# FreditorK/Tensor-Train-Interior-Point-Method

Measured on AMD Instinct MI355X. Metric: sec/IPM-iter (AMEn KKT solve), maxcut dim=10 r=1; MFMA util% on core-contract, lower is better.
Workload: dtype f64

## Files before the change

### tensor-train-interior-point-method_amd/csrc/ttk_dense.hip

```cpp
#include <hip/hip_runtime.h>

#include "ttk_common.h"
#include "ttk_internal.h"

namespace {

constexpr int NB = 32;
constexpr int GT = 32, GK = 16;

typedef double double4_t __attribute__((ext_vector_type(4)));

template <bool TA, bool TB>
__global__ __launch_bounds__(256) void gemm_strided_kernel(const double *__restrict__ A, int lda,
                                                           const double *__restrict__ B, int ldb,
                                                           double *__restrict__ C, int ldc, int M, int N, int K,
                                                           double alpha, double beta, int lower_only) {
  const int n0 = blockIdx.x * GT, m0 = blockIdx.y * GT;
  if (lower_only && n0 > m0 + GT - 1) return;
  __shared__ double As[GK][GT + 1];
  __shared__ double Bs[GK][GT + 1];
  const int tid = threadIdx.x, lane = tid & 63, wid = tid >> 6;
  const int wr = wid >> 1, wc = wid & 1;
  const int l_mn = tid & 31, l_k = tid >> 5;
  const bool am = m0 + l_mn < M, bn = n0 + l_mn < N;
// ... 82 lines not shown
}

__global__ __launch_bounds__(256) void panel_trsm_kernel(double *A, int n, int k0, int kb, const int *status) {
  __shared__ double Ls[NB][NB + 1];
  if (*status) return;
  const int tid = threadIdx.x;
  ttk::staged_copy<4>(kb * kb, tid, 256, [&](int e) { return A[(int64_t)(k0 + e / kb) * n + k0 + e % kb]; },
                      [&](int e, double v) { Ls[e / kb][e % kb] = v; });
  __syncthreads();
  const int r = k0 + kb + blockIdx.x * 256 + tid;
  if (r >= n) return;
  double *a = A + (int64_t)r * n + k0;
  double x[NB];
#pragma unroll
  for (int j = 0; j < NB; ++j) x[j] = j < kb ? a[j] : 0.0;
#pragma unroll
  for (int j = 0; j < NB; ++j) {
    if (j < kb) {
      double s = x[j];
#pragma unroll
      for (int c = 0; c < NB; ++c)
        if (c < j) s -= x[c] * Ls[j][c];
      x[j] = s / Ls[j][j];
    }
  }
#pragma unroll
  for (int j = 0; j < NB; ++j)
    if (j < kb) a[j] = x[j];
}

__global__ __launch_bounds__(256) void zero_upper_kernel(double *A, int n, const int *status) {
  if (*status) return;
  const int64_t e = blockIdx.x * (int64_t)256 + threadIdx.x;
  if (e >= (int64_t)n * n) return;
  const int i = (int)(e / n), c = (int)(e % n);
  if (c > i) A[e] = 0.0;
}

__global__ __launch_bounds__(256) void trsm_diag_kernel(const double *__restrict__ L, int n, double *B, int nrhs,
                                                        int ldb, int r0, int kb, int trans) {
  __shared__ double Ls[NB][NB + 1];
  const int tid = threadIdx.x;
  ttk::staged_copy<4>(
      kb * kb, tid, 256,
      [&](int e) {
        const int i = e / kb, j = e - i * kb;
        return trans ? L[(int64_t)(r0 + j) * n + r0 + i] : L[(int64_t)(r0 + i) * n + r0 + j];
      },
      [&](int e, double v) { Ls[e / kb][e % kb] = v; });
  __syncthreads();
  const int c = blockIdx.x * 256 + tid;
  if (c >= nrhs) return;
  double x[NB];
#pragma unroll
  for (int j = 0; j < NB; ++j) x[j] = j < kb ? B[(int64_t)(r0 + j) * ldb + c] : 0.0;
  if (!trans) {
#pragma unroll
    for (int j = 0; j < NB; ++j) {
      if (j < kb) {
        double s = x[j];
#pragma unroll
        for (int q = 0; q < NB; ++q)
          if (q < j) s -= Ls[j][q] * x[q];
        x[j] = s / Ls[j][j];
      }
    }
  } else {
#pragma unroll
    for (int jj = NB - 1; jj >= 0; --jj) {
      if (jj < kb) {
        double s = x[jj];
#pragma unroll
        for (int q = 0; q < NB; ++q)
          if (q > jj && q < kb) s -= Ls[jj][q] * x[q];
        x[jj] = s / Ls[jj][jj];
      }
    }
  }
#pragma unroll
  for (int j = 0; j < NB; ++j)
    if (j < kb) B[(int64_t)(r0 + j) * ldb + c] = x[j];
}



__global__ __launch_bounds__(256) void colsum_kernel(const double *__restrict__ A, int n, double *__restrict__ out) {
  const int c = blockIdx.x * 256 + threadIdx.x;
  if (c >= n) return;
  out[c] = ttk::sum_ahead<8>(n, [&](int r) { return fabs(A[(int64_t)r * n + c]); }, 0.0);
}

__device__ __forceinline__ void panel_row_update(double *__restrict__ pi, const double *__restrict__ prow, int c,
                                                 int kb, double inv) {
  const double l = pi[c] * inv;
  pi[c] = l;
#pragma unroll 8
  for (int cc = c + 1; cc < kb; ++cc) pi[cc] -= l * prow[cc];
}

__global__ __launch_bounds__(1024) void getf2_panel_kernel(double *A, int n, int k0, int kb, int *piv, int *status) {
  __shared__ double wv[16];
  __shared__ int wi[16];
  __shared__ int s_p;
  const int tid = threadIdx.x, lane = tid & 63, wid = tid >> 6;
  for (int c = 0; c < kb; ++c) {
    const int j = k0 + c;
    double best = -1.0;
    int bi = j;
    for (int i = j + tid; i < n; i += 1024) {
      const double v = fabs(A[(int64_t)i * n + j]);
      if (v > best) {
        best = v;
        bi = i;
      }
    }
    ttk::wave_argmax(best, bi);
    if (lane == 0) {
      wv[wid] = best;
      wi[wid] = bi;
    }
    __syncthreads();
    if (tid == 0) {
      double b = wv[0];
      int p = wi[0];
      for (int w = 1; w < 16; ++w)
        if (wv[w] > b || (wv[w] == b && wi[w] < p)) {
          b = wv[w];
          p = wi[w];
        }
      s_p = p;
      piv[j] = p;
    }
    __syncthreads();
    const int p = s_p;
    if (p != j && tid < kb) {
      double *a = A + (int64_t)j * n + k0 + tid, *b = A + (int64_t)p * n + k0 + tid;
      const double t = *a;
      *a = *b;
      *b = t;
    }
    __syncthreads();
    const double d = A[(int64_t)j * n + j];
    if (d == 0.0) {
      if (tid == 0 && *status == 0) *status = j + 1;
      continue;
    }
    const double inv = 1.0 / d;
    const double *prow = A + (int64_t)j * n + k0;
    for (int i = j + 1 + tid; i < n; i += 1024) panel_row_update(A + (int64_t)i * n + k0, prow, c, kb, inv);
    __syncthreads();
  }
}

__global__ __launch_bounds__(1024) void getf2_panel_lds_kernel(double *A, int n, int k0, int kb, int *piv,
                                                               int *status) {
  extern __shared__ double P[];
  __shared__ double wv[16];
  __shared__ int wi[16];
  __shared__ int s_p;
  const int tid = threadIdx.x, lane = tid & 63, wid = tid >> 6, nt = blockDim.x, nw = nt >> 6;
  const int rows = n - k0, ld = kb + 1;
  ttk::staged_copy<8>(rows * kb, tid, nt, [&](int e) { return A[(int64_t)(k0 + e / kb) * n + k0 + e % kb]; },
                      [&](int e, double v) { P[(e / kb) * ld + e % kb] = v; });
  __syncthreads();
  for (int c = 0; c < kb; ++c) {
    double best = -1.0;
// ... 592 lines not shown
        hipLaunchKernelGGL((getf2_panel_reg_kernel<8, 3>), dim3(1), dim3(1024), 0, st, A, n, k0, kb, piv, status);
      else
        hipLaunchKernelGGL((getf2_panel_reg_kernel<8, 4>), dim3(1), dim3(1024), 0, st, A, n, k0, kb, piv, status);
    } else if (pshm <= 150000) {
      if (pshm > 65536)
        (void)hipFuncSetAttribute(reinterpret_cast<const void *>(getf2_panel_lds_kernel),
                                  hipFuncAttributeMaxDynamicSharedMemorySize, (int)pshm);
      const int ntp = g_lu_panel_narrow ? ((n - k0 + 63) / 64 * 64 < 1024 ? (n - k0 + 63) / 64 * 64 : 1024) : 1024;
      hipLaunchKernelGGL(getf2_panel_lds_kernel, dim3(1), dim3(ntp), pshm, st, A, n, k0, kb, piv, status);
    } else {
      hipLaunchKernelGGL(getf2_panel_kernel, dim3(1), dim3(1024), 0, st, A, n, k0, kb, piv, status);
    }
    const int rest = n - k0 - kb;
    if (g_lu_swap_u12) {
      if (n - kb > 0)
        hipLaunchKernelGGL(lu_swap_u12_kernel, dim3((n - kb + 255) / 256), dim3(256), 0, st, A, n, k0, kb, piv);
    } else {
      hipLaunchKernelGGL(laswp_kernel, dim3((n + 255) / 256), dim3(256), 0, st, A, n, k0, kb, piv);
      if (rest > 0)
        hipLaunchKernelGGL(lu_u12_kernel, dim3((rest + 255) / 256), dim3(256), 0, st, A, n, k0, kb);
    }
    if (rest > 0) {
      dim3 grid((rest + GT - 1) / GT, (rest + GT - 1) / GT);
      hipLaunchKernelGGL((gemm_strided_kernel<false, false>), grid, dim3(256), 0, st,
                         A + (int64_t)(k0 + kb) * n + k0, n, A + (int64_t)k0 * n + k0 + kb, n,
                         A + (int64_t)(k0 + kb) * n + k0 + kb, n, rest, rest, kb, -1.0, 1.0, 0);
    }
    TTK_LAUNCH_CHECK();
    k0 += kb;
  }
  if (want_rcond == 1) return lu_rcond_launch(st, A, n, piv, colsum, status, rcond);
  return TTK_OK;
}

int lu_rcond_launch(hipStream_t st, const double *LU, int n, const int *piv, const double *colsum, const int *status,
                    double *rcond) {
  const size_t shm_perm = 3 * (size_t)n * sizeof(double) + 2 * (size_t)n * sizeof(int);
  const int use_perm = shm_perm <= 140000;
  const size_t shm = use_perm ? shm_perm : 2 * (size_t)n * sizeof(double) + (size_t)n * sizeof(int);
  if (shm > 65536)
    (void)hipFuncSetAttribute(reinterpret_cast<const void *>(lu_rcond_kernel),
                              hipFuncAttributeMaxDynamicSharedMemorySize, (int)shm);
  const int exact = ttk::ctx().knob[TTK_KNOB_RCOND_EXACT] != 0;
  hipLaunchKernelGGL(lu_rcond_kernel, dim3(1), dim3(1024), shm, st, LU, n, piv, colsum, status, rcond, use_perm,
                     exact);
  TTK_LAUNCH_CHECK();
  return TTK_OK;
}

int lu_solve_cols(hipStream_t st, const double *LU, int n, const int *piv, double *B, int nrhs, int ldb) {
  const size_t shm = (size_t)n * (sizeof(double) + sizeof(int));
  if (shm > 65536)
    (void)hipFuncSetAttribute(reinterpret_cast<const void *>(lu_solve_cols_kernel),
                              hipFuncAttributeMaxDynamicSharedMemorySize, (int)shm);
  hipLaunchKernelGGL(lu_solve_cols_kernel, dim3(nrhs), dim3(1024), shm, st, LU, n, piv, B, ldb);
  TTK_LAUNCH_CHECK();
  return TTK_OK;
}


int cholesky_blocked(hipStream_t st, double *A, int n, int *status) {
  TTK_HIP(hipMemsetAsync(status, 0, sizeof(int), st));
  for (int k0 = 0; k0 < n; k0 += NB) {
    const int kb = n - k0 < NB ? n - k0 : NB;
    hipLaunchKernelGGL(potf2_block_kernel, dim3(1), dim3(256), 0, st, A, n, k0, kb, status);
    const int rest = n - k0 - kb;
    if (rest > 0) {
      hipLaunchKernelGGL(panel_trsm_kernel, dim3((rest + 255) / 256), dim3(256), 0, st, A, n, k0, kb, status);
      double *L21 = A + (int64_t)(k0 + kb) * n + k0;
      double *A22 = A + (int64_t)(k0 + kb) * n + k0 + kb;
      dim3 grid((rest + GT - 1) / GT, (rest + GT - 1) / GT);
      hipLaunchKernelGGL((gemm_strided_kernel<false, true>), grid, dim3(256), 0, st, L21, n, L21, n, A22, n, rest,
                         rest, kb, -1.0, 1.0, 1);
    }
    TTK_LAUNCH_CHECK();
  }
  hipLaunchKernelGGL(zero_upper_kernel, dim3((unsigned)(((int64_t)n * n + 255) / 256)), dim3(256), 0, st, A, n,
                     status);
  TTK_LAUNCH_CHECK();
  return TTK_OK;
}

int trsm_blocked(hipStream_t st, const double *L, int n, double *B, int nrhs, int ldb, int trans) {
  for (int s = 0; s < n; s += NB) {
    const int kb = n - s < NB ? n - s : NB;
    const int r0 = trans ? n - s - kb : s;
    hipLaunchKernelGGL(trsm_diag_kernel, dim3((nrhs + 255) / 256), dim3(256), 0, st, L, n, B, nrhs, ldb, r0, kb,
                       trans);
    const int rest = n - s - kb;
    if (rest > 0) {
      dim3 grid((nrhs + GT - 1) / GT, (rest + GT - 1) / GT);
      if (!trans) {
        hipLaunchKernelGGL((gemm_strided_kernel<false, false>), grid, dim3(256), 0, st,
                           L + (int64_t)(r0 + kb) * n + r0, n, B + (int64_t)r0 * ldb, ldb,
                           B + (int64_t)(r0 + kb) * ldb, ldb, rest, nrhs, kb, -1.0, 1.0, 0);
      } else {
        hipLaunchKernelGGL((gemm_strided_kernel<true, false>), grid, dim3(256), 0, st, L + (int64_t)r0 * n, n,
                           B + (int64_t)r0 * ldb, ldb, B, ldb, rest, nrhs, kb, -1.0, 1.0, 0);
      }
    }
    TTK_LAUNCH_CHECK();
  }
  return TTK_OK;
}

}
```

### tensor-train-interior-point-method_amd/csrc/ttk_host.hip

```cpp
#include <cmath>
#include <tuple>
#include <cstring>
#include <vector>

#include "ttk_common.h"
#include "ttk_internal.h"

namespace {

struct Scratch {
  hipStream_t st;
  std::vector<void *> ptrs;
  double *base = nullptr;
  int64_t cap = 0, used = 0;
  static int64_t slot(int64_t n) { return ((n > 0 ? n : 1) + 31) & ~(int64_t)31; }
  explicit Scratch(hipStream_t s, int64_t capacity = 0) : st(s) {
    void *p = nullptr;
    if (capacity > 0 && hipMallocAsync(&p, (size_t)capacity * sizeof(double), st) == hipSuccess) {
      ptrs.push_back(p);
      base = static_cast<double *>(p);
      cap = capacity;
    }
  }
  double *get(int64_t n) {
// ... 67 lines not shown
}

View v3(const double *p, int64_t a, int64_t b, int64_t c) { return View{p, 3, {a, b, c}, {b * c, c, 1}}; }

int einsum_out(hipStream_t st, const char *eq, std::initializer_list<View> ops, double *out, int ond,
               const int64_t *ost, double alpha, double beta) {
  int64_t d[1 + 8 * 10 + 2 + 8];
  int k = 0;
  d[k++] = (int64_t)ops.size();
  for (const View &o : ops) {
    d[k++] = reinterpret_cast<int64_t>(o.p);
    d[k++] = o.nd;
    for (int i = 0; i < o.nd; ++i) d[k++] = o.sh[i];
    for (int i = 0; i < o.nd; ++i) d[k++] = o.st[i];
  }
  d[k++] = 1;
  d[k++] = ond;
  for (int i = 0; i < ond; ++i) d[k++] = ost[i];
  return ttk_einsum(st, eq, d, out, alpha, beta);
}

}

extern "C" {

int ttk_dense_schur_solve(ttk_ctx ctx, int64_t r, int64_t n, int64_t R, const ttk_local_block *blk,
                          const double *rhs, const double *inv_I, double *sol, double *rcond_out) {
  ttk::CtxScope scope(ctx);
  hipStream_t st = ttk::ctx().stream;
  if (rcond_out) *rcond_out = NAN;
  const int64_t m = r * n * R;
  if (r < 1 || n < 1 || R < 1 || !blk || !rhs || !inv_I || !sol || m > (1 << 20)) {
    ttk::set_error("ttk_dense_schur_solve: bad arguments");
    return TTK_ERR_ARG;
  }
  static const char *ASSEMBLE = "lsr,smnS,LSR->lmLrnR", *APPLY = "lsr,smnS,LSR,rnR->lmL",
                    *APPLY_T = "lsr,smnS,LSR,lmL->rnR", *MATMUL = "ik,kj->ij";
  enum { B00, B01, B21, B22 };
  auto ops3 = [&](int b) {
    const ttk_local_block &q = blk[b];
    return std::make_tuple(v3(q.L, r, q.s, r),
                           View{q.A, 4, {q.s, n, n, q.S}, {q.a_strides[0], q.a_strides[1], q.a_strides[2], q.a_strides[3]}},
                           v3(q.R, R, q.S, R));
  };
  Scratch sc(st, 7 * Scratch::slot(m) + 5 * Scratch::slot(m * m) + Scratch::slot(2 * m + 16) + Scratch::slot(m / 2 + 1));
  double *rd = sc.get(m), *rc = sc.get(m), *rp = sc.get(m), *LXI = sc.get(m * m), *Leq = sc.get(m * m),
         *LZ = sc.get(m * m), *t = sc.get(m), *bvec = sc.get(m), *T1 = sc.get(m * m), *Am = sc.get(m * m),
         *t2 = sc.get(m), *t3 = sc.get(m), *work = sc.get(2 * m + 16);
  int *piv = reinterpret_cast<int *>(sc.get(m / 2 + 1));
  if (!rd || !rc || !rp || !LXI || !Leq || !LZ || !t || !bvec || !T1 || !Am || !t2 || !t3 || !work || !piv) {
    ttk::set_error("ttk_dense_schur_solve: scratch allocation failed");
    return TTK_ERR_HIP;
  }
  const int64_t sh3[3] = {r, n, R}, st_blk[3] = {3 * n * R, R, 1}, st_c[3] = {n * R, R, 1};
  const int64_t out6[6] = {n * R * m, R * m, m, n * R, R, 1};
  const int64_t mm[2] = {m, m}, s_mat[2] = {m, 1}, s_row[2] = {0, 1}, out2[2] = {1, 1};
  auto col = [&](int j) { return rhs + j * n * R; };
  int rc_ = TTK_OK;
#define STEP(x)              \
  do {                       \
    if (rc_ == TTK_OK) rc_ = (x); \
  } while (0)
  STEP(ttk_copy_nd(st, col(1), rd, 3, sh3, st_blk, st_c, 1.0, 0.0));
  STEP(ttk_copy_nd(st, col(2), rc, 3, sh3, st_blk, st_c, 1.0, 0.0));
  STEP(ttk_copy_nd(st, col(0), rp, 3, sh3, st_blk, st_c, 1.0, 0.0));
  {
    auto [a, b, c] = ops3(B22);
    STEP(einsum(st, ASSEMBLE, {a, b, c}, LXI));
  }
  STEP(ttk_mul_nd(st, LXI, inv_I, LXI, 2, mm, s_mat, s_row, s_mat, 1.0, 0.0));
  {
    auto [a, b, c] = ops3(B01);
    STEP(einsum(st, ASSEMBLE, {a, b, c}, Leq));
  }
  {
    auto [a, b, c] = ops3(B21);
    STEP(einsum(st, ASSEMBLE, {a, b, c}, LZ));
  }
  if (rc_) return rc_;
  rc_ = ttk_cholesky_sync(st, LZ, (int)m);
  if (rc_) return rc_;
  STEP(hipMemcpyAsync(t, rc, m * sizeof(double), hipMemcpyDeviceToDevice, st) ? TTK_ERR_HIP : 0);
  STEP(einsum_out(st, MATMUL, {mat(LXI, m, m), mat(rd, m, 1)}, t, 2, out2, -1.0, 1.0));
  STEP(ttk_trsm_lower(st, LZ, (int)m, t, 1, 1, 0));
  STEP(ttk_trsm_lower(st, LZ, (int)m, t, 1, 1, 1));
  STEP(hipMemcpyAsync(bvec, rp, m * sizeof(double), hipMemcpyDeviceToDevice, st) ? TTK_ERR_HIP : 0);
  STEP(einsum_out(st, MATMUL, {mat(Leq, m, m), mat(t, m, 1)}, bvec, 2, out2, -1.0, 1.0));
  STEP(ttk_trsm_lower(st, LZ, (int)m, LXI, (int)m, (int)m, 0));
  STEP(ttk_trsm_lower(st, LZ, (int)m, LXI, (int)m, (int)m, 1));
  STEP(einsum(st, MATMUL, {mat(LXI, m, m), View{Leq, 2, {m, m}, {1, m}}}, T1));
  STEP(einsum(st, MATMUL, {mat(Leq, m, m), mat(T1, m, m)}, Am));
  {
    auto [a, b, c] = ops3(B00);
    STEP(einsum_out(st, ASSEMBLE, {a, b, c}, Am, 6, out6, 1.0, 1.0));
  }
  STEP(ttk_add_diag(st, Am, (int)m, (int)m, 1e-11));
  if (rc_) return rc_;
  int forked = 0;
  rc_ = ttk::lu_factor_fork_rcond(st, Am, (int)m, piv, work, &forked);
  if (rc_) return rc_;
  STEP(ttk_lu_solve(st, Am, (int)m, piv, bvec, 1, 1));
  double *s0 = sol, *s1 = sol + n * R, *s2 = sol + 2 * n * R;
  STEP(ttk_copy_nd(st, bvec, s0, 3, sh3, st_c, st_blk, 1.0, 0.0));
  STEP(hipMemcpyAsync(t2, rd, m * sizeof(double), hipMemcpyDeviceToDevice, st) ? TTK_ERR_HIP : 0);
  {
    auto [a, b, c] = ops3(B01);
    const View x{s0, 3, {r, n, R}, {st_blk[0], st_blk[1], st_blk[2]}};
    STEP(einsum_out(st, APPLY_T, {a, b, c, x}, t2, 3, st_c, -1.0, 1.0));
  }
  STEP(ttk_mul_nd(st, t2, inv_I, s2, 3, sh3, st_c, st_c, st_blk, 1.0, 0.0));
  STEP(hipMemcpyAsync(t3, rc, m * sizeof(double), hipMemcpyDeviceToDevice, st) ? TTK_ERR_HIP : 0);
  {
    auto [a, b, c] = ops3(B22);
    const View x{s2, 3, {r, n, R}, {st_blk[0], st_blk[1], st_blk[2]}};
    STEP(einsum_out(st, APPLY, {a, b, c, x}, t3, 3, st_c, -1.0, 1.0));
  }
  STEP(ttk_trsm_lower(st, LZ, (int)m, t3, 1, 1, 0));
  STEP(ttk_trsm_lower(st, LZ, (int)m, t3, 1, 1, 1));
  STEP(ttk_copy_nd(st, t3, s1, 3, sh3, st_c, st_blk, 1.0, 0.0));
#undef STEP
  if (forked && ttk::lu_rcond_join(st)) return TTK_ERR_HIP;
  int lu_info = 0;
  double rcond = 0.0;
  if (hipMemcpyAsync(&lu_info, ttk::ctx().status, sizeof(int), hipMemcpyDeviceToHost, st) ||
      hipMemcpyAsync(&rcond, ttk::ctx().rcond, sizeof(double), hipMemcpyDeviceToHost, st))
    return TTK_ERR_HIP;
  ttk::note_sync();
  if (hipStreamSynchronize(st)) return TTK_ERR_HIP;
  if (rcond_out) *rcond_out = rcond;
  if (lu_info) {
    ttk::set_error("Matrix is singular (zero pivot at %d).", lu_info);
    return TTK_ERR_SINGULAR;
  }
  if (rcond < 0.5 * 2.220446049250313e-16) return TTK_ILL_CONDITIONED;
  return rc_;
}

int ttk_dense_schur_solve_ineq(ttk_ctx ctx, int64_t r, int64_t n, int64_t R, const ttk_local_block *blk,
                               const double *rhs, const double *inv_I, double *sol) {
  ttk::CtxScope scope(ctx);
  hipStream_t st = ttk::ctx().stream;
  const int64_t m = r * n * R;
  if (r < 1 || n < 1 || R < 1 || !blk || !rhs || !inv_I || !sol || m > (1 << 20)) {
    ttk::set_error("ttk_dense_schur_solve_ineq: bad arguments");
    return TTK_ERR_ARG;
  }
  static const char *ASSEMBLE = "lsr,smnS,LSR->lmLrnR", *APPLY = "lsr,smnS,LSR,rnR->lmL",
                    *APPLY_T = "lsr,smnS,LSR,lmL->rnR", *MATMUL = "ik,kj->ij";
  enum { B00, B01, B21, B22, B31, B33 };
  auto ops3 = [&](int b) {
    const ttk_local_block &q = blk[b];
    return std::make_tuple(v3(q.L, r, q.s, r),
                           View{q.A, 4, {q.s, n, n, q.S}, {q.a_strides[0], q.a_strides[1], q.a_strides[2], q.a_strides[3]}},
                           v3(q.R, R, q.S, R));
  };
  Scratch sc(st, 12 * Scratch::slot(m) + 12 * Scratch::slot(m * m) + Scratch::slot(2 * m + 16) +
                     2 * Scratch::slot(m / 2 + 1));
  double *rp = sc.get(m), *rd = sc.get(m), *rc = sc.get(m), *rt = sc.get(m), *LZ = sc.get(m * m),
         *LZ_rc = sc.get(m), *LZ_LX = sc.get(m * m), *Leq = sc.get(m * m), *Top = sc.get(m * m),
         *LZ_LXI = sc.get(m * m), *w = sc.get(m), *u = sc.get(m), *v = sc.get(m), *Am = sc.get(m * m),
         *T = sc.get(m * m), *Dm = sc.get(m * m), *TL = sc.get(m * m), *Top2 = sc.get(m * m), *Leq2 = sc.get(m * m),
         *Dv = sc.get(m), *DT = sc.get(m * m), *y = sc.get(m), *t2 = sc.get(m), *t3 = sc.get(m),
         *work = sc.get(2 * m + 16);
  int *dpiv = reinterpret_cast<int *>(sc.get(m / 2 + 1)), *piv = reinterpret_cast<int *>(sc.get(m / 2 + 1));
  for (double *p : {rp, rd, rc, rt, LZ, LZ_rc, LZ_LX, Leq, Top, LZ_LXI, w, u, v, Am, T, Dm, TL, Top2, Leq2, Dv, DT, y,
                    t2, t3, work})
    if (!p || !dpiv || !piv) {
      ttk::set_error("ttk_dense_schur_solve_ineq: scratch allocation failed");
      return TTK_ERR_HIP;
    }
  const int64_t sh3[3] = {r, n, R}, st_blk[3] = {4 * n * R, R, 1}, st_c[3] = {n * R, R, 1};
  const int64_t mm[2] = {m, m}, s_mat[2] = {m, 1}, s_row[2] = {0, 1}, out1[2] = {1, 1}, outm[2] = {m, 1};
// ... 228 lines not shown
```

### tensor-train-interior-point-method_amd/csrc/ttk_internal.h

```cpp
#ifndef TTK_INTERNAL_H
#define TTK_INTERNAL_H

#include <hip/hip_runtime.h>

#include <cstdlib>

#include "../../include/ttk.h"

namespace ttk {
inline int env_int(const char *name, int dflt) {
  const char *v = std::getenv(name);
  return v ? std::atoi(v) : dflt;
}
struct UpSlot {
  double *p = nullptr;
  size_t n = 0;
  hipEvent_t ev = nullptr;
  bool pending = false;
};
constexpr int UP_SLOTS = 64;

struct Ctx {
  hipStream_t stream = nullptr;
  double *scratch = nullptr;
  int64_t scratch_n = 0;
  void *batch = nullptr;
  double *splitk = nullptr;
  int64_t splitk_n = 0;
  double *dev_scalar = nullptr;
  void *schur = nullptr;
  double *schur_w = nullptr;
  int64_t schur_wcap = 0;
  unsigned *dep = nullptr;
  unsigned dep_total = 0;
  unsigned tick_total = 0;
  unsigned *splitk_cnt = nullptr;
  double *lgmres = nullptr;
  int64_t lgmres_n = 0;
  int *status = nullptr;
  double *rcond = nullptr;
  double *mapped_h = nullptr, *mapped_d = nullptr;
  size_t mapped_n = 0;
  UpSlot up[UP_SLOTS];
  int up_next = 0;
  hipStream_t side = nullptr;
  hipEvent_t ev_fork = nullptr, ev_join = nullptr;
  int knob[TTK_KNOB_COUNT] = {env_int("TTK_FUSED_APPLY", 1) != 0 ? 1 : 0, env_int("TTK_FUSED_MFMA", 1) != 0 ? 1 : 0,
                              env_int("TTK_SPLITK", 1) != 0 ? 1 : 0,
                              env_int("TTK_SPLITK_MINK", 128) > 0 ? env_int("TTK_SPLITK_MINK", 128) : 128,
                              env_int("TTK_LGMRES_MW_MIN", 16384), env_int("TTK_MFMA_CSPLIT", 1) != 0 ? 1 : 0,
                              env_int("TTK_APPLY_DUAL", 1) != 0 ? 1 : 0, env_int("TTK_RCOND_EXACT", 0) != 0 ? 1 : 0,
                              env_int("TTK_SCHUR_ONE", 1) != 0 ? 1 : 0, env_int("TTK_ARNOLDI_ONE", 0) != 0 ? 1 : 0,
                              env_int("TTK_SCHUR_PREP", 1) != 0 ? 1 : 0, env_int("TTK_SPLITK_FUSED", 1) != 0 ? 1 : 0,
                              env_int("TTK_TRI_HOIST", 1) != 0 ? 1 : 0, env_int("TTK_TRI_ONE", 0),
                              env_int("TTK_TRI_PERSIST", 0) != 0 ? 1 : 0, env_int("TTK_SYEV_WAVES8", 1) != 0 ? 1 : 0,
                              env_int("TTK_BT_STAGE", 1) != 0 ? 1 : 0};
};
Ctx &ctx();
Ctx *ctx_swap(Ctx *c);
void schur_release(Ctx &c);
int presize_splitk();
int presize_lgmres();
int presize_schur();
}

struct ttk_ctx_s {
  ttk::Ctx c;
};

namespace ttk {
struct CtxScope {
  Ctx *prev;
  bool on;
  explicit CtxScope(ttk_ctx_s *h) : prev(nullptr), on(h != nullptr) {
    if (on) prev = ctx_swap(&h->c);
  }
  ~CtxScope() {
    if (on) ctx_swap(prev);
  }
};
void ctx_free_einsum(Ctx &c);

int cholesky_blocked(hipStream_t st, double *A, int n, int *status);
int trsm_blocked(hipStream_t st, const double *L, int n, double *B, int nrhs, int ldb, int trans);
int lu_blocked(hipStream_t st, double *A, int n, int *piv, double *work, int *status, double *rcond, int want_rcond);
int lu_rcond_launch(hipStream_t st, const double *LU, int n, const int *piv, const double *colsum, const int *status,
                    double *rcond);
int lu_factor_fork_rcond(hipStream_t st, double *A, int n, int *piv, double *work, int *forked);
int lu_rcond_join(hipStream_t st);
int lu_solve_cols(hipStream_t st, const double *LU, int n, const int *piv, double *B, int nrhs, int ldb);
int qr_colmajor(void *stream, const double *At, int m, int n, double *Qt, double *R, double *work);

struct GemmProblem {
  const double *A, *B;
  double *C;
  const int64_t *offs;
  int nb, M, N, K;
  double alpha, beta;
};
bool gemm_groupable(int nb, int M, int N, int K);
int gemm_group(hipStream_t st, const GemmProblem *p, int n);
int batch_barrier(void *stream);
int schur_apply(void *stream, int64_t handle, const double *v, double *out);
}

#endif
```

### tensor-train-interior-point-method_amd/csrc/ttk_linalg.hip

```cpp
#include <math.h>
#include <stdlib.h>

#include <array>
#include <chrono>
#include <cstdio>
#include <cstring>
#include <map>
#include <mutex>

#include "ttk_common.h"
#include "ttk_internal.h"

namespace {

constexpr double EPS = 2.220446049250313e-16;
__device__ unsigned long long g_dbg[8];

constexpr int LDS_DOUBLES = 20000;

__device__ __forceinline__ void rr_pair(int P, int r, int k, int &p, int &q) {
  const int P1 = P - 1;
  if (k == 0) {
    p = r;
    q = P1;
// ... 2915 lines not shown
  if (use_lds) {
    allow_big_lds(qr_kernel<true>, shm);
    hipLaunchKernelGGL(qr_kernel<true>, dim3(1), dim3(nt), shm, TTK_STREAM(stream), A, m, n, Q, R, work, use_lds, colmajor);
  } else {
    allow_big_lds(qr_kernel<false>, shm);
    hipLaunchKernelGGL(qr_kernel<false>, dim3(1), dim3(nt), shm, TTK_STREAM(stream), A, m, n, Q, R, work, use_lds, colmajor);
  }
  TTK_LAUNCH_CHECK();
  return TTK_OK;
}

static int g_dense_block_min = 96;
static int g_lu_block_min = getenv("TTK_LU_BLOCK_MIN") ? atoi(getenv("TTK_LU_BLOCK_MIN")) : 32;

int ttk_dense_set_block_min(int n) {
  const int old = g_dense_block_min;
  g_dense_block_min = n;
  return old;
}

int ttk_cholesky_sync(void *stream, double *A, int n) {
  if (int brc = ttk::batch_barrier(stream)) return brc;
  if (ensure_status()) {
    ttk::set_error("ttk_cholesky_sync: status alloc failed");
    return TTK_ERR_HIP;
  }
  LinalgScope scope_(TTK_STREAM(stream), 4, n, n, n >= g_dense_block_min);
  if (n >= g_dense_block_min) {
    const int rc = ttk::cholesky_blocked(TTK_STREAM(stream), A, n, ttk::ctx().status);
    if (rc) return rc;
  } else {
    hipLaunchKernelGGL(chol_kernel, dim3(1), dim3(1024), 0, TTK_STREAM(stream), A, n, ttk::ctx().status);
    TTK_LAUNCH_CHECK();
  }
  int st = 0;
  TTK_HIP(hipMemcpyAsync(&st, ttk::ctx().status, sizeof(int), hipMemcpyDeviceToHost, TTK_STREAM(stream)));
  ttk::note_sync();
  TTK_HIP(hipStreamSynchronize(TTK_STREAM(stream)));
  if (st) {
    ttk::set_error("%d-th leading minor of the array is not positive definite", st);
    return TTK_ERR_NOT_PD;
  }
  return TTK_OK;
}

int ttk_trsm_lower(void *stream, const double *L, int n, double *B, int nrhs, int ldb, int trans) {
  if (int brc = ttk::batch_barrier(stream)) return brc;
  if (n <= 0 || nrhs <= 0) return TTK_OK;
  if (n >= g_dense_block_min) return ttk::trsm_blocked(TTK_STREAM(stream), L, n, B, nrhs, ldb, trans);
  hipLaunchKernelGGL(trsm_kernel, dim3((nrhs + 63) / 64), dim3(256), 0, TTK_STREAM(stream), L, n, B, nrhs, ldb, trans);
  TTK_LAUNCH_CHECK();
  return TTK_OK;
}

int ttk_lu_sync(void *stream, double *A, int n, int *piv, double *work, double *rcond_out) {
  if (int brc = ttk::batch_barrier(stream)) return brc;
  if (ensure_status()) {
    ttk::set_error("ttk_lu_sync: status alloc failed");
    return TTK_ERR_HIP;
  }
  LinalgScope scope_(TTK_STREAM(stream), 3, n, n, n >= g_lu_block_min && n <= 7000);
  if (n >= g_lu_block_min && n <= 7000) {
    const int rc = ttk::lu_blocked(TTK_STREAM(stream), A, n, piv, work, ttk::ctx().status, ttk::ctx().rcond, 1);
    if (rc) return rc;
  } else {
    hipLaunchKernelGGL(lu_kernel, dim3(1), dim3(1024), 0, TTK_STREAM(stream), A, n, piv, work, ttk::ctx().status, ttk::ctx().rcond);
    TTK_LAUNCH_CHECK();
  }
  int st = 0;
  TTK_HIP(hipMemcpyAsync(&st, ttk::ctx().status, sizeof(int), hipMemcpyDeviceToHost, TTK_STREAM(stream)));
  TTK_HIP(hipMemcpyAsync(rcond_out, ttk::ctx().rcond, sizeof(double), hipMemcpyDeviceToHost, TTK_STREAM(stream)));
  ttk::note_sync();
  TTK_HIP(hipStreamSynchronize(TTK_STREAM(stream)));
  if (st) {
    ttk::set_error("Matrix is singular (zero pivot at %d).", st);
    return TTK_ERR_SINGULAR;
  }
  return TTK_OK;
}

}

namespace ttk {
int lu_factor_fork_rcond(hipStream_t st, double *A, int n, int *piv, double *work, int *forked) {
  *forked = 0;
  if (ensure_status()) {
    set_error("lu_factor_fork_rcond: status alloc failed");
    return TTK_ERR_HIP;
  }
  Ctx &c = ctx();
  LinalgScope scope_(st, 3, n, n, n >= g_lu_block_min && n <= 7000 ? 2 : 3);
  if (!(n >= g_lu_block_min && n <= 7000)) {
    hipLaunchKernelGGL(lu_kernel, dim3(1), dim3(1024), 0, st, A, n, piv, work, c.status, c.rcond);
    TTK_LAUNCH_CHECK();
    return TTK_OK;
  }
  static const int fork_on = getenv("TTK_LU_FORK") ? atoi(getenv("TTK_LU_FORK")) : 1;
  if (!fork_on) {
    const int rc = lu_blocked(st, A, n, piv, work, c.status, c.rcond, 1);
    return rc;
  }
  if (!c.side) {
    TTK_HIP(hipStreamCreateWithFlags(&c.side, hipStreamNonBlocking));
    TTK_HIP(hipEventCreateWithFlags(&c.ev_fork, hipEventDisableTiming));
    TTK_HIP(hipEventCreateWithFlags(&c.ev_join, hipEventDisableTiming));
  }
  const int rc = lu_blocked(st, A, n, piv, work, c.status, c.rcond, 2);
  if (rc) return rc;
  TTK_HIP(hipEventRecord(c.ev_fork, st));
  TTK_HIP(hipStreamWaitEvent(c.side, c.ev_fork, 0));
  const int rr = lu_rcond_launch(c.side, A, n, piv, work, c.status, c.rcond);
  if (rr) return rr;
  TTK_HIP(hipEventRecord(c.ev_join, c.side));
  *forked = 1;
  return TTK_OK;
}

int lu_rcond_join(hipStream_t st) {
  TTK_HIP(hipStreamWaitEvent(st, ctx().ev_join, 0));
  return TTK_OK;
}
}

extern "C" {

int ttk_lu_solve(void *stream, const double *LU, int n, const int *piv, double *B, int nrhs, int ldb) {
  if (int brc = ttk::batch_barrier(stream)) return brc;
  if (n >= g_lu_block_min && n <= 12000 && nrhs <= 8 && nrhs > 0) return ttk::lu_solve_cols(TTK_STREAM(stream), LU, n, piv, B, nrhs, ldb);
  if (n <= 0 || nrhs <= 0) return TTK_OK;
  hipLaunchKernelGGL(lu_solve_kernel, dim3((nrhs + 63) / 64), dim3(256), 0, TTK_STREAM(stream), LU, n, piv, B, nrhs, ldb);
  TTK_LAUNCH_CHECK();
  return TTK_OK;
}

int64_t ttk_syev_work(int n) { return 2 * (int64_t)n * n + 2 * (n / 2 + 1) + 2 * (int64_t)n + 16; }

int ttk_syev(void *stream, double *A, int n, double *ev, double *W, double *work) {
  if (int brc = ttk::batch_barrier(stream)) return brc;
  if (n <= 0) {
    ttk::set_error("ttk_syev: empty matrix");
    return TTK_ERR_ARG;
  }
  const int64_t need = ttk_syev_work(n);
  const int use_lds = need <= LDS_DOUBLES;
  const size_t shm = use_lds ? need * sizeof(double) : 0;
  allow_big_lds(syev_kernel, shm);
  hipLaunchKernelGGL(syev_kernel, dim3(1), dim3(1024), shm, TTK_STREAM(stream), A, n, ev, W, work, use_lds);
  TTK_LAUNCH_CHECK();
  return TTK_OK;
}

int ttk_debug_counters(unsigned long long *out, int reset) {
  TTK_HIP(hipMemcpyFromSymbol(out, HIP_SYMBOL(g_dbg), sizeof(g_dbg)));
  if (reset) {
    unsigned long long z[8] = {0, 0, 0, 0, 0, 0, 0, 0};
    TTK_HIP(hipMemcpyToSymbol(HIP_SYMBOL(g_dbg), z, sizeof(z)));
  }
  return TTK_OK;
}

static int g_syev_small = 1;

int ttk_syev_set_small(int on) {
  const int old = g_syev_small;
  g_syev_small = on;
  return old;
}

int64_t ttk_syev_extreme_work(int n) {
  if (n <= 0) return 0;
  const int64_t fused = (int64_t)n * n + 18 * (int64_t)n + 64;
  const int64_t need = syev_extreme_need(n);
  return need > fused ? need : fused;
}

static int g_syev_fused_max = TRI_FUSED_MAX;
static int g_syev_small_wide = getenv("TTK_SYEV_WIDE") ? atoi(getenv("TTK_SYEV_WIDE")) : 64;
static int g_tri_rows = getenv("TTK_TRI_ROWS") ? atoi(getenv("TTK_TRI_ROWS")) : 4;

int ttk_syev_set_fused_max(int n) {
  const int old = g_syev_fused_max;
  g_syev_fused_max = n < TRI_FUSED_MAX ? n : TRI_FUSED_MAX;
  return old;
}

int ttk_syev_extreme(void *stream, const double *A, int n, int which, double *ev, double *vec, double *work) {
  if (int brc = ttk::batch_barrier(stream)) return brc;
  if (n <= 0 || (which != 0 && which != 1)) {
    ttk::set_error("ttk_syev_extreme: bad arguments");
// ... 101 lines not shown
```

Before: 0.08266.

## Fuse single-RHS triangular solves into one MFMA kernel and overlap on side stream

Adds a single-workgroup trsm kernel for one right-hand side that keeps x in LDS. Wave 0 solves each diagonal block with lane shuffles while the other waves prefetch tiles of L and apply the off-diagonal update with f64 MFMA. This replaces the many per-block diag/gemm launches for vector solves. The host also moves the two vector solves onto a side stream so they overlap the matrix-RHS solves, then joins before the result is used. The costs are a single CU doing the whole vector solve, and extra event record/wait overhead.

```diff
diff --git a/tensor-train-interior-point-method_amd/csrc/ttk_dense.hip b/tensor-train-interior-point-method_amd/csrc/ttk_dense.hip
--- a/tensor-train-interior-point-method_amd/csrc/ttk_dense.hip
+++ b/tensor-train-interior-point-method_amd/csrc/ttk_dense.hip
@@ -188,6 +188,146 @@
     if (j < kb) B[(int64_t)(r0 + j) * ldb + c] = x[j];
 }
 
+constexpr int VEC_NT = 1024, VEC_NW = VEC_NT / 64 - 1;
+constexpr int VEC_MAX_N = 1536;
+
+__global__ __launch_bounds__(VEC_NT) void trsm_vec_kernel(const double *__restrict__ L, int n, double *B, int ldb,
+                                                          int trans) {
+  extern __shared__ double vsh[];
+  double *xs = vsh;
+  double(*Ls)[NB][NB + 1] = reinterpret_cast<double(*)[NB][NB + 1]>(vsh + n);
+  double(*Tw)[16][NB + 1] = reinterpret_cast<double(*)[16][NB + 1]>(vsh + n + 2 * NB * (NB + 1));
+  const int tid = threadIdx.x, lane = tid & 63, wid = tid >> 6;
+  const int lrow = lane & 15, lk = lane >> 4;
+  for (int i = tid; i < n; i += VEC_NT) xs[i] = B[(int64_t)i * ldb];
+  auto diag_ld = [&](int s) -> double {
+    const int s0 = s * NB;
+    if (s0 >= n) return 0.0;
+    const int kb = n - s0 < NB ? n - s0 : NB, r0 = trans ? n - s0 - kb : s0;
+    if (tid >= kb * kb) return 0.0;
+    const int i = tid / kb, j = tid - i * kb;
+    return trans ? L[(int64_t)(r0 + j) * n + r0 + i] : L[(int64_t)(r0 + i) * n + r0 + j];
+  };
+  auto diag_st = [&](int s, double v) {
+    const int s0 = s * NB;
+    if (s0 >= n) return;
+    const int kb = n - s0 < NB ? n - s0 : NB;
+    if (tid < kb * kb) Ls[s & 1][tid / kb][tid % kb] = v;
+  };
+  diag_st(0, diag_ld(0));
+  __syncthreads();
+  for (int s = 0; s * NB < n; ++s) {
+    const int s0 = s * NB, kb = n - s0 < NB ? n - s0 : NB, r0 = trans ? n - s0 - kb : s0;
+    const int rest = n - s0 - kb, base = trans ? 0 : r0 + kb;
+    const int ntile = (rest + 15) / 16;
+    const double(*Ld)[NB + 1] = Ls[s & 1];
+    auto ld_tile = [&](int t, double(&a)[8]) {
+#pragma unroll
+      for (int g = 0; g < 8; ++g) {
+        if (trans) {
+          const int row = t * 16 + lrow, k = g * 4 + lk;
+          a[g] = (row < rest && k < kb) ? L[(int64_t)(r0 + k) * n + base + row] : 0.0;
+        } else {
+          const int row = t * 16 + 2 * g + (lane >> 5), k = lane & 31;
+          a[g] = (row < rest && k < kb) ? L[(int64_t)(base + row) * n + r0 + k] : 0.0;
+        }
+      }
+    };
+    auto to_mfma = [&](double(&a)[8]) {
+      if (trans) return;
+      double(*T)[NB + 1] = Tw[wid - 1];
+      __builtin_amdgcn_fence(__ATOMIC_RELEASE, "wavefront");
+      __builtin_amdgcn_wave_barrier();
+#pragma unroll
+      for (int g = 0; g < 8; ++g) T[2 * g + (lane >> 5)][lane & 31] = a[g];
+      __builtin_amdgcn_fence(__ATOMIC_RELEASE, "wavefront");
+      __builtin_amdgcn_wave_barrier();
+      __builtin_amdgcn_fence(__ATOMIC_ACQUIRE, "wavefront");
+#pragma unroll
+      for (int g = 0; g < 8; ++g) a[g] = T[lrow][g * 4 + lk];
+    };
+    const double dnext = diag_ld(s + 1);
+    double a[8] = {0.0, 0.0, 0.0, 0.0, 0.0, 0.0, 0.0, 0.0};
+    if (wid != 0) {
+      if (wid - 1 < ntile) ld_tile(wid - 1, a);
+    } else {
+      if (!trans) {
+        const int hl = lane & 31;
+        double lr[NB];
+#pragma unroll
+        for (int p = 0; p < NB; ++p) lr[p] = (p < hl && hl < kb) ? Ld[hl][p] : 0.0;
+        const double d = hl < kb ? Ld[hl][hl] : 1.0;
+        double xq = hl < kb ? xs[r0 + hl] : 0.0;
+#pragma unroll
+        for (int p = 0; p < NB; ++p) {
+          if (p < kb) {
+            if (hl == p) xq = xq / d;
+            const double xp = ttk::readlane_d(xq, p);
+            if (hl > p) xq -= lr[p] * xp;
+          }
+        }
+        if (lane < kb) xs[r0 + lane] = xq;
+      } else {
+        const int hl = lane & 31;
+        double lr[NB], sx[NB];
+#pragma unroll
+        for (int q = 0; q < NB; ++q) {
+          lr[q] = (q > hl && q < kb && hl < kb) ? Ld[hl][q] : 0.0;
+          sx[q] = 0.0;
+        }
+        const double d = hl < kb ? Ld[hl][hl] : 1.0;
+        double xq = hl < kb ? xs[r0 + hl] : 0.0;
+#pragma unroll
+        for (int jj = NB - 1; jj >= 0; --jj) {
+          if (jj < kb) {
+            double t = xq;
+#pragma unroll
+            for (int q = 0; q < NB; ++q)
+              if (q > jj) t -= lr[q] * sx[q];
+            t = t / d;
+            if (hl == jj) xq = t;
+            sx[jj] = ttk::readlane_d(xq, jj);
+          }
+        }
+        if (lane < kb) xs[r0 + lane] = xq;
+      }
+    }
+    diag_st(s + 1, dnext);
+    __syncthreads();
+    for (int t = wid != 0 ? wid - 1 : ntile; t < ntile; t += VEC_NW) {
+      double an[8] = {0.0, 0.0, 0.0, 0.0, 0.0, 0.0, 0.0, 0.0};
+      if (t + VEC_NW < ntile) ld_tile(t + VEC_NW, an);
+      to_mfma(a);
+      double4_t acc = {0.0, 0.0, 0.0, 0.0};
+#pragma unroll
+      for (int g = 0; g < GK / 4; ++g) {
+        const int k = g * 4 + lk;
+        const double b = (lrow == 0 && k < kb) ? xs[r0 + k] : 0.0;
+        acc = __builtin_amdgcn_mfma_f64_16x16x4f64(a[g], b, acc, 0, 0, 0);
+      }
+      if (kb > GK) {
+#pragma unroll
+        for (int g = GK / 4; g < 2 * GK / 4; ++g) {
+          const int k = g * 4 + lk;
+          const double b = (lrow == 0 && k < kb) ? xs[r0 + k] : 0.0;
+          acc = __builtin_amdgcn_mfma_f64_16x16x4f64(a[g], b, acc, 0, 0, 0);
+        }
+      }
+      if (lrow == 0) {
+#pragma unroll
+        for (int r = 0; r < 4; ++r) {
+          const int row = t * 16 + lk + 4 * r;
+          if (row < rest) xs[base + row] = 1.0 * xs[base + row] + (-1.0) * acc[r];
+        }
+      }
+#pragma unroll
+      for (int g = 0; g < 8; ++g) a[g] = an[g];
+    }
+    __syncthreads();
+  }
+  for (int i = tid; i < n; i += VEC_NT) B[(int64_t)i * ldb] = xs[i];
+}
+
 
 
 __global__ __launch_bounds__(256) void colsum_kernel(const double *__restrict__ A, int n, double *__restrict__ out) {
@@ -946,11 +1086,22 @@
 }
 
 int trsm_blocked(hipStream_t st, const double *L, int n, double *B, int nrhs, int ldb, int trans) {
+  constexpr size_t vshm_max = ((size_t)VEC_MAX_N + (2 * NB + 16 * VEC_NW) * (NB + 1)) * sizeof(double);
+  static_assert(vshm_max <= 150000, "x, two diagonal blocks and the waves' tiles must fit the LDS");
+  if (nrhs == 1 && n <= VEC_MAX_N) {
+    (void)hipFuncSetAttribute(reinterpret_cast<const void *>(trsm_vec_kernel),
+                              hipFuncAttributeMaxDynamicSharedMemorySize, (int)vshm_max);
+    const size_t vshm = ((size_t)n + (2 * NB + 16 * VEC_NW) * (NB + 1)) * sizeof(double);
+    hipLaunchKernelGGL(trsm_vec_kernel, dim3(1), dim3(VEC_NT), vshm, st, L, n, B, ldb, trans);
+    TTK_LAUNCH_CHECK();
+    return TTK_OK;
+  }
   for (int s = 0; s < n; s += NB) {
     const int kb = n - s < NB ? n - s : NB;
     const int r0 = trans ? n - s - kb : s;
     hipLaunchKernelGGL(trsm_diag_kernel, dim3((nrhs + 255) / 256), dim3(256), 0, st, L, n, B, nrhs, ldb, r0, kb,
                        trans);
+    TTK_LAUNCH_CHECK();
     const int rest = n - s - kb;
     if (rest > 0) {
       dim3 grid((nrhs + GT - 1) / GT, (rest + GT - 1) / GT);
@@ -962,8 +1113,8 @@
         hipLaunchKernelGGL((gemm_strided_kernel<true, false>), grid, dim3(256), 0, st, L + (int64_t)r0 * n, n,
                            B + (int64_t)r0 * ldb, ldb, B, ldb, rest, nrhs, kb, -1.0, 1.0, 0);
       }
-    }
-    TTK_LAUNCH_CHECK();
+      TTK_LAUNCH_CHECK();
+    }
   }
   return TTK_OK;
 }
diff --git a/tensor-train-interior-point-method_amd/csrc/ttk_host.hip b/tensor-train-interior-point-method_amd/csrc/ttk_host.hip
--- a/tensor-train-interior-point-method_amd/csrc/ttk_host.hip
+++ b/tensor-train-interior-point-method_amd/csrc/ttk_host.hip
@@ -173,12 +173,18 @@
   if (rc_) return rc_;
   STEP(hipMemcpyAsync(t, rc, m * sizeof(double), hipMemcpyDeviceToDevice, st) ? TTK_ERR_HIP : 0);
   STEP(einsum_out(st, MATMUL, {mat(LXI, m, m), mat(rd, m, 1)}, t, 2, out2, -1.0, 1.0));
-  STEP(ttk_trsm_lower(st, LZ, (int)m, t, 1, 1, 0));
-  STEP(ttk_trsm_lower(st, LZ, (int)m, t, 1, 1, 1));
+  hipStream_t side = nullptr;
+  STEP(ttk::side_fork(st, &side));
+  if (rc_) return rc_;
+  hipStream_t ts = side ? side : st;
+  STEP(ttk_trsm_lower(ts, LZ, (int)m, t, 1, 1, 0));
+  STEP(ttk_trsm_lower(ts, LZ, (int)m, t, 1, 1, 1));
+  if (side && ttk::side_done()) return TTK_ERR_HIP;
+  STEP(ttk_trsm_lower(st, LZ, (int)m, LXI, (int)m, (int)m, 0));
+  STEP(ttk_trsm_lower(st, LZ, (int)m, LXI, (int)m, (int)m, 1));
+  if (side && ttk::lu_rcond_join(st)) return TTK_ERR_HIP;
   STEP(hipMemcpyAsync(bvec, rp, m * sizeof(double), hipMemcpyDeviceToDevice, st) ? TTK_ERR_HIP : 0);
   STEP(einsum_out(st, MATMUL, {mat(Leq, m, m), mat(t, m, 1)}, bvec, 2, out2, -1.0, 1.0));
-  STEP(ttk_trsm_lower(st, LZ, (int)m, LXI, (int)m, (int)m, 0));
-  STEP(ttk_trsm_lower(st, LZ, (int)m, LXI, (int)m, (int)m, 1));
   STEP(einsum(st, MATMUL, {mat(LXI, m, m), View{Leq, 2, {m, m}, {1, m}}}, T1));
   STEP(einsum(st, MATMUL, {mat(Leq, m, m), mat(T1, m, m)}, Am));
   {
diff --git a/tensor-train-interior-point-method_amd/csrc/ttk_internal.h b/tensor-train-interior-point-method_amd/csrc/ttk_internal.h
--- a/tensor-train-interior-point-method_amd/csrc/ttk_internal.h
+++ b/tensor-train-interior-point-method_amd/csrc/ttk_internal.h
@@ -88,6 +88,8 @@
                     double *rcond);
 int lu_factor_fork_rcond(hipStream_t st, double *A, int n, int *piv, double *work, int *forked);
 int lu_rcond_join(hipStream_t st);
+int side_fork(hipStream_t st, hipStream_t *side);
+int side_done();
 int lu_solve_cols(hipStream_t st, const double *LU, int n, const int *piv, double *B, int nrhs, int ldb);
 int qr_colmajor(void *stream, const double *At, int m, int n, double *Qt, double *R, double *work);
 
diff --git a/tensor-train-interior-point-method_amd/csrc/ttk_linalg.hip b/tensor-train-interior-point-method_amd/csrc/ttk_linalg.hip
--- a/tensor-train-interior-point-method_amd/csrc/ttk_linalg.hip
+++ b/tensor-train-interior-point-method_amd/csrc/ttk_linalg.hip
@@ -3021,6 +3021,36 @@
 }
 
 namespace ttk {
+static int lu_fork_on() {
+  static const int on = getenv("TTK_LU_FORK") ? atoi(getenv("TTK_LU_FORK")) : 1;
+  return on;
+}
+
+static int side_ensure(Ctx &c) {
+  if (!c.side) {
+    TTK_HIP(hipStreamCreateWithFlags(&c.side, hipStreamNonBlocking));
+    TTK_HIP(hipEventCreateWithFlags(&c.ev_fork, hipEventDisableTiming));
+    TTK_HIP(hipEventCreateWithFlags(&c.ev_join, hipEventDisableTiming));
+  }
+  return TTK_OK;
+}
+
+int side_fork(hipStream_t st, hipStream_t *side) {
+  *side = nullptr;
+  if (!lu_fork_on()) return TTK_OK;
+  Ctx &c = ctx();
+  if (int rc = side_ensure(c)) return rc;
+  TTK_HIP(hipEventRecord(c.ev_fork, st));
+  TTK_HIP(hipStreamWaitEvent(c.side, c.ev_fork, 0));
+  *side = c.side;
+  return TTK_OK;
+}
+
+int side_done() {
+  TTK_HIP(hipEventRecord(ctx().ev_join, ctx().side));
+  return TTK_OK;
+}
+
 int lu_factor_fork_rcond(hipStream_t st, double *A, int n, int *piv, double *work, int *forked) {
   *forked = 0;
   if (ensure_status()) {
@@ -3034,16 +3064,11 @@
     TTK_LAUNCH_CHECK();
     return TTK_OK;
   }
-  static const int fork_on = getenv("TTK_LU_FORK") ? atoi(getenv("TTK_LU_FORK")) : 1;
-  if (!fork_on) {
+  if (!lu_fork_on()) {
     const int rc = lu_blocked(st, A, n, piv, work, c.status, c.rcond, 1);
     return rc;
   }
-  if (!c.side) {
-    TTK_HIP(hipStreamCreateWithFlags(&c.side, hipStreamNonBlocking));
-    TTK_HIP(hipEventCreateWithFlags(&c.ev_fork, hipEventDisableTiming));
-    TTK_HIP(hipEventCreateWithFlags(&c.ev_join, hipEventDisableTiming));
-  }
+  if (int rs = side_ensure(c)) return rs;
   const int rc = lu_blocked(st, A, n, piv, work, c.status, c.rcond, 2);
   if (rc) return rc;
   TTK_HIP(hipEventRecord(c.ev_fork, st));
```

Measured after the change: 0.08455. 1.02x slower.
